# tigarcia/firedancer

Measured on AMD Instinct MI355X. Metric: ed25519 verifies/sec at 1/8 GPUs; % INT32 VALU roofline; p99 batch latency, higher is better.
Workload: dtype int32

## Files before the change

firedancer_amd/csrc/fd_ed25519_kernels.hip:

```cpp
#include <hip/hip_runtime.h>
#include "fd25519_dsm.h"
#include "fd25519_ge4.h"
#include "fd25519_sc.h"
#include "fd_sha512_dev.h"
#define FD_HALF_FN __device__ static inline
#define FD_HALF_RCP(y) __builtin_amdgcn_rcp(y)
#define FD_HALF_RCPF(y) __builtin_amdgcn_rcpf(y)
#include "fd25519_half.h"



#define FD_PF_FAIL  1u
#define FD_PF_SMALL 2u
#define FD_HF_DNEG  1u
#define FD_HF_FULL  2u


FD_DEV uint32_t nblk_bucket(uint32_t sz) {
  const uint32_t b = (sz + 208u) >> 7;
  return b < (FD_ED25519_SORT_BUCKETS - 1) ? b : (FD_ED25519_SORT_BUCKETS - 1);
}

#define FD_SORT_PER_THREAD 16
#define FD_SORT_PER_BLOCK (256 * FD_SORT_PER_THREAD)
// ... 108 lines not shown
  hash_finish(p, j, dig, S);
}

__global__ void __launch_bounds__(256, FD_ED25519_HASH_WAVES_PER_SIMD)
fd_ed25519_hash_kernel(fd_ed25519_verify_params_t p) {
  const uint64_t t = (uint64_t)blockIdx.x * blockDim.x + threadIdx.x;
  if (t >= p.n) return;
  hash_one(p, p.perm ? (uint64_t)p.perm[t] : t);
}

FD_DEV void decode_one(const fd_ed25519_verify_params_t& p, int which , uint64_t j) {
  const uint64_t i = p.base + j;
  uint32_t s[8];
  {
    const uint4* src = which ? reinterpret_cast<const uint4*>(p.sigs + 64 * i)
                             : reinterpret_cast<const uint4*>(p.pubs + 32 * i);
    const uint4 q0 = src[0], q1 = src[1];
    s[0] = q0.x; s[1] = q0.y; s[2] = q0.z; s[3] = q0.w; s[4] = q1.x; s[5] = q1.y; s[6] = q1.z; s[7] = q1.w;
  }
  decoded_pt d;
  ge_decode(d, s, !p.codes_portable);
  int32_t* dst = p.pts + (uint64_t)which * 20 * p.cap + j;
#pragma unroll
  for (int l = 0; l < 10; l++) {
    dst[(uint64_t)l * p.cap] = d.x.v[l];
    dst[(uint64_t)(10 + l) * p.cap] = d.y.v[l];
  }
  p.pflag[(uint64_t)which * p.cap + j] = (uint8_t)((d.fail ? FD_PF_FAIL : 0u) | (d.small ? FD_PF_SMALL : 0u));
}

__global__ void __launch_bounds__(256, FD_ED25519_DECODE_WAVES_PER_SIMD)
fd_ed25519_decode_kernel(fd_ed25519_verify_params_t p) {
  const uint64_t t = (uint64_t)blockIdx.x * blockDim.x + threadIdx.x;
  if (t >= 2 * p.n) return;
  const int which = t >= p.n;
  decode_one(p, which, which ? t - p.n : t);
}

FD_DEV void load_fe(fe& x, const int32_t* src, uint64_t cap) {
#pragma unroll
  for (int l = 0; l < 10; l++) x.v[l] = src[(uint64_t)l * cap];
}

FD_DEV void load_pt(fe& x, fe& y, const fd_ed25519_verify_params_t& p, int which, uint64_t j) {
  const int32_t* src = p.pts + (uint64_t)which * 20 * p.cap + j;
  load_fe(x, src, p.cap);
  load_fe(y, src + 10 * p.cap, p.cap);
}

#define FD_PENDING 1
FD_DEV int precheck(const fd_ed25519_verify_params_t& p, uint64_t j) {
  const uint32_t s_ok = p.sflag[j];
  const uint32_t af = p.pflag[j], rf = p.pflag[p.cap + j];
  if (!s_ok) return FD_ED25519_ERR_SIG;
  if (af & FD_PF_FAIL) return p.codes_portable ? FD_ED25519_ERR_PUBKEY : FD_ED25519_ERR_SIG;
  if (rf & FD_PF_FAIL) return FD_ED25519_ERR_SIG;
  if (af & FD_PF_SMALL) return FD_ED25519_ERR_PUBKEY;
  if (rf & FD_PF_SMALL) return FD_ED25519_ERR_SIG;
  return FD_PENDING;
}

template <bool NT>
FD_DEV void table_store(int4* tab, int e, ge_cached c) {
  if (NT) fe_neg(c.T2d, c.T2d);
  atab_store(tab, e, c);
}

__device__ const int4 fd_ident_cached[10] = {{1, 0, 0, 0}, {0, 0, 0, 0}, {0, 0, 1, 0}, {0, 0, 0, 0}, {0, 0, 0, 0},
                                             {2, 0, 0, 0}, {0, 0, 0, 0}, {0, 0, 0, 0}, {0, 0, 0, 0}, {0, 0, 0, 0}};

template <bool IDENT>
FD_DEV const int4* tab_entry(const int4* tab, int e) {
  const int a = e < 0 ? -e : e;
  if (IDENT) return a == 0 ? fd_ident_cached : tab + (a - 1) * 10;
  return tab + a * 10;
}

template <bool NT, bool IDENT = false>
FD_DEV void table_build(int4* tab, const fe& x, const fe& y, bool negate) {
  ge_p3 P0;
  fe xn;
  fe_neg(xn, x);
  fe_select(P0.X, x, xn, negate);
  P0.Y = y;
  fe_1(P0.Z);
  fe_mul(P0.T, P0.X, y);
  ge_cached c1, c;
  if (!IDENT) {
    c.YplusX = P0.Z; c.YminusX = P0.Z; fe_add(c.Z2, P0.Z, P0.Z); fe_0(c.T2d);
    atab_store(tab, 0, c);
  }
  ge_p3_to_cached(c1, P0);
  table_store<NT>(tab, IDENT ? 0 : 1, c1);
  ge_precomp pre;
  pre.yplusx = c1.YplusX; pre.yminusx = c1.YminusX; pre.xy2d = c1.T2d;
  ge_p3 cur = P0;
  ge_p1p1 sum;
#pragma clang loop unroll(disable)
  for (int e = 2; e <= 8; e++) {
    ge_madd(sum, cur, pre);
    ge_p1p1_to_p3_uxyt(cur, sum);
    ge_p3_to_cached<true>(c, cur);
    table_store<NT>(tab, IDENT ? e - 1 : e, c);
  }
}

FD_DEV void table_add(ge_p1p1& Rt, const ge_p3& P, const int4* tab, int e) {
  ge_cached c;
  atab_load(c, tab, e < 0 ? -e : e);
  ge_cached_cneg(c, e < 0);
  ge_add(Rt, P, c);
}

FD_DEV void btab_add(ge_p1p1& Rt, const ge_p3& P, ge_precomp& b, int f) {
  ge_precomp_cneg(b, f < 0);
  ge_madd(Rt, P, b);
}


FD_DEV bool half_pair_ok(const uint32_t (&k)[8], const uint32_t (&c)[FD_HALF_TW], const uint32_t (&dm)[FD_HALF_TW],
                         int dneg, int dbits) {
  uint32_t x[16];
#pragma unroll
  for (int w = 0; w < 16; w++) x[w] = 0u;
#pragma unroll
  for (int a = 0; a < FD_HALF_TW; a++) {
    uint64_t carry = 0;
#pragma unroll
    for (int b = 0; b < 8; b++) {
      const uint64_t t = (uint64_t)dm[a] * k[b] + x[a + b] + carry;
      x[a + b] = (uint32_t)t;
      carry = t >> 32;
    }
    x[a + 8] = (uint32_t)carry;
  }
  const uint32_t n8l[8] = FD_HALF_N8L;
  uint32_t add[8];
  {
    uint64_t br = 0;
#pragma unroll
    for (int w = 0; w < 8; w++) {
      const uint32_t cv = w < FD_HALF_TW ? c[w] : 0u;
      const uint64_t t = (uint64_t)n8l[w] - cv - br;
      br = (t >> 63) & 1u;
      add[w] = dneg ? cv : (uint32_t)t;
    }
  }
  {
    uint64_t carry = 0;
#pragma unroll
    for (int w = 0; w < 15; w++) {
      const uint64_t t = (uint64_t)x[w] + (w < 8 ? add[w] : 0u) + carry;
      x[w] = (uint32_t)t;
      carry = t >> 32;
    }
  }
  const uint32_t low = x[0] & 7u;
#pragma unroll
  for (int w = 0; w < 15; w++) x[w] = __builtin_amdgcn_alignbit(x[w + 1], x[w], 3);
  x[15] >>= 3;
  uint32_t r[8];
  sc_reduce512(r, x);
  uint32_t nz = low;
#pragma unroll
  for (int w = 0; w < 8; w++) nz |= r[w];
  return nz == 0u && (dm[0] & 1u) && fd_half_bitlen<FD_HALF_TW>(c) <= FD_HALF_BITS &&
         fd_half_bitlen<FD_HALF_TW>(dm) <= dbits;
}

#ifndef FD_ED25519_AB_LDS_BASE
#define FD_ED25519_AB_LDS_BASE 0
#endif
#ifndef FD_ED25519_HALF_FAULT
#define FD_ED25519_HALF_FAULT 0
#endif

FD_DEV int half_scalars_checked(const uint32_t (&k)[8], uint32_t (&c)[FD_HALF_TW], uint32_t (&dm)[FD_HALF_TW],
                                int* dneg, int dbits, uint64_t tag) {
  const int found = fd_half_scalars(k, c, dm, dneg, dbits);
#if FD_ED25519_HALF_FAULT
  {
    const uint32_t h = (uint32_t)(tag * 0x9E3779B97F4A7C15ull >> 32);
    const uint32_t sel = h >> 29, w = (h >> 8) & 3u, b = h & 31u;
#pragma unroll
    for (int i = 0; i < 4; i++) {
      if (sel == 1u && i == (int)w) c[i] ^= 1u << b;
      if (sel == 2u && i == (int)w) dm[i] ^= (i == 0 && b == 0) ? 2u : (1u << b);
    }
  }
#else
  (void)tag;
#endif
  return found && half_pair_ok(k, c, dm, *dneg, dbits);
}


FD_DEV void scalar_one(const fd_ed25519_verify_params_t& p, uint64_t j) {
  const uint64_t i = p.base + j;
  uint32_t k[8], S[8];
#pragma unroll
  for (int w = 0; w < 8; w++) k[w] = p.k[(uint64_t)w * p.cap + j];
  {
    const uint4* sg = reinterpret_cast<const uint4*>(p.sigs + 64 * i);
    const uint4 q2 = sg[2], q3 = sg[3];
    S[0] = q2.x; S[1] = q2.y; S[2] = q2.z; S[3] = q2.w; S[4] = q3.x; S[5] = q3.y; S[6] = q3.z; S[7] = q3.w;
  }
  uint32_t cw[FD_HALF_TW], dm[FD_HALF_TW];
  int dneg = 0;
  int ok = half_scalars_checked(k, cw, dm, &dneg, p.half_dbits, j);
  if (!p.sflag[j]) ok = 1;

  uint32_t sp[8];
  {
    uint32_t prod[16];
#pragma unroll
    for (int w = 0; w < 16; w++) prod[w] = 0u;
#pragma unroll
    for (int a = 0; a < FD_HALF_TW; a++) {
      uint64_t carry = 0;
#pragma unroll
      for (int b = 0; b < 8; b++) {
        const uint64_t t = (uint64_t)dm[a] * S[b] + prod[a + b] + carry;
        prod[a + b] = (uint32_t)t;
        carry = t >> 32;
      }
      prod[a + 8] = (uint32_t)carry;
    }
    sc_reduce512(sp, prod);
    if (dneg) {
      const uint32_t l[8] = {0x5cf5d3edu, 0x5812631au, 0xa2f79cd6u, 0x14def9deu, 0u, 0u, 0u, 0x10000000u};
      uint32_t nz = 0;
#pragma unroll
      for (int w = 0; w < 8; w++) nz |= sp[w];
      uint64_t br = 0;
#pragma unroll
      for (int w = 0; w < 8; w++) {
        const uint64_t t = (uint64_t)l[w] - sp[w] - br;
        br = (t >> 63) & 1u;
        sp[w] = nz ? (uint32_t)t : 0u;
      }
    }
  }
  uint32_t* hs = p.hs + j;
  const uint64_t c = p.cap;
  static_assert(FD_ED25519_BTABW_SHIFT == 144, "s_lo is words 0..3 and the low half of word 4");
#pragma unroll
  for (int w = 0; w < 5; w++) {
    hs[(uint64_t)w * c] = cw[w];
    hs[(uint64_t)(5 + w) * c] = dm[w];
    hs[(uint64_t)(10 + w) * c] = w < 4 ? sp[w] : (sp[4] & 0xffffu);
  }
#pragma unroll
  for (int w = 0; w < 4; w++)
    hs[(uint64_t)(15 + w) * c] = __builtin_amdgcn_alignbit(w + 5 < 8 ? sp[w + 5] : 0u, sp[w + 4], 16);
  p.hflag[j] = (uint8_t)((dneg ? FD_HF_DNEG : 0u) | (ok ? 0u : FD_HF_FULL));
  if (!ok && !p.small) {
    const uint32_t slot = atomicAdd(p.fix_cnt, 1u);
    p.fix_list[slot] = (uint32_t)j;
  }
}

__global__ void __launch_bounds__(256, FD_ED25519_SCALAR_WAVES_PER_SIMD)
fd_ed25519_scalar_kernel(fd_ed25519_verify_params_t p) {
  const uint64_t j = (uint64_t)blockIdx.x * blockDim.x + threadIdx.x;
  if (j >= p.n) return;
  scalar_one(p, j);
}

__global__ void __launch_bounds__(192) fd_ed25519_prep_kernel(fd_ed25519_verify_params_t p) {
  const uint32_t w = threadIdx.x >> 6;
  const uint64_t t = (uint64_t)blockIdx.x * 64u + (threadIdx.x & 63u);
  if (t >= p.n) return;
  if (w == 0) {
    const uint64_t j = p.perm ? (uint64_t)p.perm[t] : t;
    hash_one(p, j);
    scalar_one(p, j);
  } else {
    decode_one(p, (int)w - 1, t);
  }
}


FD_DEV void load_hs(uint32_t (&x)[5], const fd_ed25519_verify_params_t& p, int row, int words, uint64_t j) {
#pragma unroll
  for (int w = 0; w < 5; w++) x[w] = w < words ? p.hs[(uint64_t)(row + w) * p.cap + j] : 0u;
}

template <int BW>
struct fd_bw {
  static constexpr int STEP   = BW / 4;
  static constexpr int LO_N   = FD_ED25519_BTABW_SHIFT / BW;
  static constexpr int HI_N   = (253 - FD_ED25519_BTABW_SHIFT + BW - 1) / BW;
  static constexpr int LO_SHL = 160 - LO_N * BW;
  static constexpr int HI_SHL = 160 - HI_N * BW;
  static_assert(BW % 4 == 0, "base digits start at window boundaries");
  static_assert(LO_N * BW == FD_ED25519_BTABW_SHIFT, "s_lo digits cover bits 0..SHIFT-1");
  static_assert(HI_N * BW >= 253 - FD_ED25519_BTABW_SHIFT, "s_hi digits cover s' >> SHIFT");
  static_assert(STEP * (LO_N - 1) <= 32, "every base digit falls within the 33 windows");
  FD_DEV static bool lo_at(int it) { return it <= STEP * (LO_N - 1) && it % STEP == 0; }
  FD_DEV static bool hi_at(int it) { return it <= STEP * (HI_N - 1) && it % STEP == 0; }
};


template <int BW>
FD_DEV int dsm_half_one(const fd_ed25519_verify_params_t& p, uint64_t j, int4* tabA, int4* tabR) {
  int code = precheck(p, j);
  const uint32_t hf = p.hflag[j];

  {
    fe x, y;
    load_pt(x, y, p, 0, j);
    table_build<true, true>(tabA, x, y, true);
    load_pt(x, y, p, 1, j);
    table_build<true, true>(tabR, x, y, !(hf & FD_HF_DNEG));
  }
  uint32_t cd[5], dd[5], ld[5], hd[5];
  int W = 33;
  {
    uint32_t x[5], t[5];
    load_hs(x, p, 5, 5, j);
    const int wl = (fd_half_bitlen<5>(x) + 4) >> 2;
#pragma unroll
    for (int w = 34; w <= (FD_HALF_DBITS_MAX + 4) / 4; w++) W += __ballot(wl >= w) != 0ull;
    const int sh = 160 - 4 * W;
    shl160v(t, x, sh); recode160<4>(dd, t);
    load_hs(x, p, 0, 5, j);  shl160v(t, x, sh); recode160<4>(cd, t);
    load_hs(x, p, 10, 5, j); shl160<fd_bw<BW>::LO_SHL>(ld, x);
    load_hs(x, p, 15, 4, j); shl160<fd_bw<BW>::HI_SHL>(hd, x);
  }
  const int4* g_btab = reinterpret_cast<const int4*>(p.btab_lo);
  const int4* g_btab2 = reinterpret_cast<const int4*>(p.btab_hi);

  ge_p3 P;
  ge_p3_0(P);
  ge_p1p1 Rt;
  ge_p2 Q;
#pragma clang loop unroll(disable)
  for (int it = W - 1; it >= 0; it--) {
    int ea = pop160<4>(cd), er = pop160<4>(dd);
    if (it == W - 1) { ea &= 15; er &= 15; }
    ge_cached ca, cr;
    const bool blo = fd_bw<BW>::lo_at(it), bhi = fd_bw<BW>::hi_at(it);
    ge_precomp b1, b2;
    atab_load(ca, tab_entry<true>(tabA, ea), 0);
    if (it != W - 1) {
#pragma clang loop unroll(disable)
      for (int dbl = 0; dbl < 4; dbl++) {
        ge_p2_dbl(Rt, Q);
        if (dbl < 3) ge_p1p1_to_p2(Q, Rt);
      }
      ge_p1p1_to_p3_u(P, Rt);
    }
    atab_load(cr, tab_entry<true>(tabR, er), 0);
    ge_cached_cneg(ca, ea < 0);
    ge_add<true>(Rt, P, ca);
    ge_p1p1_to_p3_u(P, Rt);
    if (blo) btab16_load(b1, g_btab, (int)pop160u<BW>(ld));
    if (bhi) btab16_load(b2, g_btab2, (int)pop160u<BW>(hd));
    ge_cached_cneg(cr, er < 0);
    ge_add<true>(Rt, P, cr);
    if (blo) {
      ge_p1p1_to_p3_uxyt(P, Rt);
      ge_madd(Rt, P, b1);
    }
    if (bhi) {
      ge_p1p1_to_p3_uxyt(P, Rt);
      ge_madd(Rt, P, b2);
    }
    ge_p1p1_to_p2(Q, Rt);
  }
  fe t;
  fe_sub(t, Q.Y, Q.Z);
  const bool ident = fe_iszero(Q.X) && fe_iszero(t);
  if (code == FD_PENDING) code = ident ? FD_ED25519_SUCCESS : FD_ED25519_ERR_MSG;
  return code;
}

#if FD_ED25519_AB_LDS_BASE
FD_DEV int dsm_half_one_lds(const fd_ed25519_verify_params_t& p, uint64_t j, int4* tabA, int4* tabR,
                            const int4* s_lo8, const int4* s_hi8) {
  int code = precheck(p, j);
  const uint32_t hf = p.hflag[j];
  {
    fe x, y;
    load_pt(x, y, p, 0, j);
    table_build<true, true>(tabA, x, y, true);
    load_pt(x, y, p, 1, j);
    table_build<true, true>(tabR, x, y, !(hf & FD_HF_DNEG));
  }
  uint32_t cd[5], dd[5], ld[5], hd[5];
  int W = 33;
  {
    uint32_t x[5], t[5], sl[5], sh[5];
    load_hs(x, p, 5, 5, j);
    const int wl = (fd_half_bitlen<5>(x) + 4) >> 2;
#pragma unroll
    for (int w = 34; w <= (FD_HALF_DBITS_MAX + 4) / 4; w++) W += __ballot(wl >= w) != 0ull;
    const int shv = 160 - 4 * W;
    shl160v(t, x, shv); recode160<4>(dd, t);
    load_hs(x, p, 0, 5, j);  shl160v(t, x, shv); recode160<4>(cd, t);
    load_hs(sl, p, 10, 5, j);
    load_hs(sh, p, 15, 4, j);
    static_assert(FD_ED25519_BTABW_SHIFT - FD_ED25519_BTAB8_SHIFT == 8, "re-split of s' by one byte");
    uint32_t lo[5] = {sl[0], sl[1], sl[2], sl[3], sl[4] & 0xffu};
    uint32_t hi[5] = {(sl[4] >> 8) | (sh[0] << 8), (sh[0] >> 24) | (sh[1] << 8), (sh[1] >> 24) | (sh[2] << 8),
                      (sh[2] >> 24) | (sh[3] << 8), sh[3] >> 24};
    shl160<160 - 17 * 8>(ld, lo);
    shl160<160 - 15 * 8>(hd, hi);
  }
  ge_p3 P;
  ge_p3_0(P);
  ge_p1p1 Rt;
  ge_p2 Q;
#pragma clang loop unroll(disable)
  for (int it = W - 1; it >= 0; it--) {
    int ea = pop160<4>(cd), er = pop160<4>(dd);
    if (it == W - 1) { ea &= 15; er &= 15; }
    ge_cached ca, cr;
    const bool blo = it <= 32 && !(it & 1), bhi = it <= 28 && !(it & 1);
    ge_precomp b1, b2;
    atab_load(ca, tab_entry<true>(tabA, ea), 0);
    if (it != W - 1) {
#pragma clang loop unroll(disable)
      for (int dbl = 0; dbl < 4; dbl++) {
        ge_p2_dbl(Rt, Q);
        if (dbl < 3) ge_p1p1_to_p2(Q, Rt);
      }
      ge_p1p1_to_p3_u(P, Rt);
    }
    atab_load(cr, tab_entry<true>(tabR, er), 0);
    ge_cached_cneg(ca, ea < 0);
    ge_add<true>(Rt, P, ca);
    ge_p1p1_to_p3_u(P, Rt);
    if (blo) btab16_load(b1, s_lo8, (int)pop160u<8>(ld));
    if (bhi) btab16_load(b2, s_hi8, (int)pop160u<8>(hd));
    ge_cached_cneg(cr, er < 0);
    ge_add<true>(Rt, P, cr);
    if (blo) {
      ge_p1p1_to_p3_uxyt(P, Rt);
      ge_madd(Rt, P, b1);
    }
    if (bhi) {
      ge_p1p1_to_p3_uxyt(P, Rt);
      ge_madd(Rt, P, b2);
    }
    ge_p1p1_to_p2(Q, Rt);
  }
  fe t;
  fe_sub(t, Q.Y, Q.Z);
  const bool ident = fe_iszero(Q.X) && fe_iszero(t);
  if (code == FD_PENDING) code = ident ? FD_ED25519_SUCCESS : FD_ED25519_ERR_MSG;
  return code;
}
#endif

FD_DEV int dsm_full_core(const fd_ed25519_verify_params_t& p, uint64_t j, int4* tabA, int code, const fe& ax,
                         const fe& ay, const fe& rx, const fe& ry) {
  const uint64_t i = p.base + j;
  table_build<false>(tabA, ax, ay, true);
  uint32_t kd[8], sd[8];
  {
    uint32_t k[8], S[8];
#pragma unroll
    for (int w = 0; w < 8; w++) k[w] = p.k[(uint64_t)w * p.cap + j];
    const uint4* sg = reinterpret_cast<const uint4*>(p.sigs + 64 * i);
    const uint4 q2 = sg[2], q3 = sg[3];
    S[0] = q2.x; S[1] = q2.y; S[2] = q2.z; S[3] = q2.w; S[4] = q3.x; S[5] = q3.y; S[6] = q3.z; S[7] = q3.w;
    recode_radix16(kd, k);
    recode_radix65536(sd, S);
  }
  const int4* g_btab = reinterpret_cast<const int4*>(p.btab16);
  ge_p3 P;
  ge_p3_0(P);
  ge_p1p1 Rt;
  ge_p2 Q;
#pragma clang loop unroll(disable)
  for (int it = 63; it >= 0; it--) {
    const bool badd = (it & 3) == 0;
    int f = 0;
    ge_precomp b;
    if (badd) {
      f = pop_digit<16>(sd);
      btab16_load(b, g_btab, f < 0 ? -f : f);
    }
    if (it != 63) {
#pragma clang loop unroll(disable)
      for (int dbl = 0; dbl < 4; dbl++) {
        ge_p2_dbl(Rt, Q);
        if (dbl < 3) ge_p1p1_to_p2(Q, Rt);
      }
      ge_p1p1_to_p3_u(P, Rt);
    }
    table_add(Rt, P, tabA, pop_digit<4>(kd));
    if (badd) {
      ge_p1p1_to_p3_uxyt(P, Rt);
      btab_add(Rt, P, b, f);
    }
    ge_p1p1_to_p2(Q, Rt);
  }
  fe t1, t2;
  fe_mul(t1, rx, Q.Z);
  fe_sub(t1, t1, Q.X);
  fe_mul(t2, ry, Q.Z);
  fe_sub(t2, t2, Q.Y);
  const bool eq = fe_iszero(t1) && fe_iszero(t2);
  if (code != FD_PENDING) return code;
  return eq ? FD_ED25519_SUCCESS : FD_ED25519_ERR_MSG;
}

FD_DEV int dsm_full_one(const fd_ed25519_verify_params_t& p, uint64_t j, int4* tabA) {
  fe ax, ay, rx, ry;
  load_pt(ax, ay, p, 0, j);
  load_pt(rx, ry, p, 1, j);
  return dsm_full_core(p, j, tabA, precheck(p, j), ax, ay, rx, ry);
}

template <int BW>
__global__ void __launch_bounds__(FD_ED25519_VERIFY_BLOCK, FD_ED25519_DSM_WAVES_PER_SIMD)
fd_ed25519_dsm_kernel(fd_ed25519_verify_params_t p) {
  const uint32_t lane = threadIdx.x & 63u;
  const uint64_t wave = ((uint64_t)blockIdx.x * blockDim.x + threadIdx.x) >> 6;
  int4* tabA = reinterpret_cast<int4*>(static_cast<char*>(p.atab) + wave * FD_ED25519_ATAB_BYTES_PER_WAVE) +
               lane * (2 * FD_ED25519_ATAB_STRIDE * 10);
  int4* tabR = tabA + FD_ED25519_ATAB_STRIDE * 10;
#if FD_ED25519_AB_LDS_BASE
  __shared__ int4 s_b8[2 * 256 * (FD_ED25519_BTAB16_STRIDE / 4)];
  {
    const int4* g_lo = reinterpret_cast<const int4*>(p.btab8_lo);
    const int4* g_hi = reinterpret_cast<const int4*>(p.btab8_hi);
    constexpr int N = 256 * (FD_ED25519_BTAB16_STRIDE / 4);
    for (int i = threadIdx.x; i < N; i += blockDim.x) { s_b8[i] = g_lo[i]; s_b8[N + i] = g_hi[i]; }
    __syncthreads();
  }
#endif
  if (p.small) {
    const uint64_t stride = (uint64_t)gridDim.x * blockDim.x;
    for (uint64_t t = (uint64_t)blockIdx.x * blockDim.x + threadIdx.x; t < p.n; t += stride)
      if (p.hflag[t] & FD_HF_FULL) p.out[p.base + t] = (int8_t)dsm_full_one(p, t, tabA);
    return;
  }
  const uint64_t nfix = *p.fix_cnt;
  const uint64_t head = (nfix + 63u) & ~(uint64_t)63u;
  const uint64_t total = head + p.n;
  for (;;) {
    uint32_t b = 0u;
    if (lane == 0u) b = atomicAdd(p.work_ctr, 64u);
    b = (uint32_t)__builtin_amdgcn_readfirstlane((int)__shfl((int)b, 0));
    if ((uint64_t)b >= total) break;
    const uint64_t t = (uint64_t)b + lane;
    if (t < nfix) {
      const uint64_t j = p.fix_list[t];
      p.out[p.base + j] = (int8_t)dsm_full_one(p, j, tabA);
    } else if (t >= head && t < total) {
      const uint64_t j = t - head;
#if FD_ED25519_AB_LDS_BASE
      if (!(p.hflag[j] & FD_HF_FULL))
        p.out[p.base + j] = (int8_t)dsm_half_one_lds(p, j, tabA, tabR, s_b8, s_b8 + 256 * (FD_ED25519_BTAB16_STRIDE / 4));
#else
      if (!(p.hflag[j] & FD_HF_FULL)) p.out[p.base + j] = (int8_t)dsm_half_one<BW>(p, j, tabA, tabR);
#endif
    }
  }
}


FD_DEV void tab4_store(int4* tab, int e, const fe& c) {
  int4* d = tab + 3 * e;
  d[0] = make_int4(c.v[0], c.v[1], c.v[2], c.v[3]);
  d[1] = make_int4(c.v[4], c.v[5], c.v[6], c.v[7]);
  d[2] = make_int4(c.v[8], c.v[9], 0, 0);
}

FD_DEV void tab4_load(fe& c, const int4* tab, int e) {
  const int4* s = tab + 3 * e;
  const int4 a = s[0], b = s[1], d = s[2];
  c.v[0] = a.x; c.v[1] = a.y; c.v[2] = a.z; c.v[3] = a.w;
  c.v[4] = b.x; c.v[5] = b.y; c.v[6] = b.z; c.v[7] = b.w;
  c.v[8] = d.x; c.v[9] = d.y;
}

FD_DEV void btab4_load(fe& c, const int32_t* g_btab, int e, const qmask_t& m) {
  const int off = m.l0 ? 10 : (m.l1 ? 0 : 20);
  const int2* s = reinterpret_cast<const int2*>(g_btab + (size_t)e * FD_ED25519_BTAB16_STRIDE + off);
#pragma unroll
  for (int q = 0; q < 5; q++) {
    const int2 x = s[q];
    c.v[2 * q] = x.x;
    c.v[2 * q + 1] = x.y;
  }
#pragma unroll
  for (int i = 0; i < 10; i++) c.v[i] = m.l3 ? (i == 0 ? 2 : 0) : c.v[i];
}

FD_DEV void table4_build(int4* tab, const fe& x, const fe& y, bool negate, const qmask_t& m) {
  fe xs, xy, p0, c1, c, r, cur;
#pragma unroll
  for (int i = 0; i < 10; i++) xs.v[i] = negate ? -x.v[i] : x.v[i];
  fe_mul(xy, xs, y);
#pragma unroll
  for (int i = 0; i < 10; i++) {
    p0.v[i] = m.l0 ? xs.v[i] : (m.l1 ? y.v[i] : (m.l2 ? (i == 0 ? 1 : 0) : xy.v[i]));
    c.v[i] = i == 0 ? (m.l2 ? 0 : (m.l3 ? 2 : 1)) : 0;
  }
  tab4_store(tab, 0, c);
  ge4_to_qc(c1, p0, m);
  tab4_store(tab, 1, c1);
  cur = p0;
#pragma clang loop unroll(disable)
  for (int e = 2; e <= 8; e++) {
    ge4_add(r, cur, c1, m);
    ge4_to_p3(cur, r);
    ge4_to_qc(c, cur, m);
    tab4_store(tab, e, c);
  }
}

template <int BW>
__global__ void __launch_bounds__(256) fd_ed25519_dsm4_kernel(fd_ed25519_verify_params_t p) {
  const uint64_t gid = (uint64_t)blockIdx.x * blockDim.x + threadIdx.x;
  const uint64_t j = gid >> 2;
  if (j >= p.n) return;
  const uint32_t hf = p.hflag[j];
  if (hf & FD_HF_FULL) return;
  const qmask_t m = quad_masks();
  int4* tabA = reinterpret_cast<int4*>(static_cast<char*>(p.atab) + gid * FD_ED25519_QUAD_LANE_BYTES);
  int4* tabR = tabA + 27;
  int code = precheck(p, j);
  {
    fe x, y;
    load_pt(x, y, p, 0, j);
    table4_build(tabA, x, y, true, m);
    load_pt(x, y, p, 1, j);
    table4_build(tabR, x, y, !(hf & FD_HF_DNEG), m);
  }
  uint32_t cd[5], dd[5], ld[5], hd[5];
  int W = 33;
  {
    uint32_t x[5], t[5];
    load_hs(x, p, 5, 5, j);
    const int wl = (fd_half_bitlen<5>(x) + 4) >> 2;
#pragma unroll
    for (int w = 34; w <= (FD_HALF_DBITS_MAX + 4) / 4; w++) W += __ballot(wl >= w) != 0ull;
    const int sh = 160 - 4 * W;
    shl160v(t, x, sh); recode160<4>(dd, t);
    load_hs(x, p, 0, 5, j);  shl160v(t, x, sh); recode160<4>(cd, t);
    load_hs(x, p, 10, 5, j); shl160<fd_bw<BW>::LO_SHL>(ld, x);
    load_hs(x, p, 15, 4, j); shl160<fd_bw<BW>::HI_SHL>(hd, x);
  }
  fe P, Rt;
#pragma unroll
  for (int i = 0; i < 10; i++) P.v[i] = (i == 0 && (m.l1 | m.l2)) ? 1 : 0;
#pragma clang loop unroll(disable)
  for (int it = W - 1; it >= 0; it--) {
    int ea = pop160<4>(cd), er = pop160<4>(dd);
    if (it == W - 1) { ea &= 15; er &= 15; }
    const bool blo = fd_bw<BW>::lo_at(it), bhi = fd_bw<BW>::hi_at(it);
    fe ca, cr, b1, b2;
    tab4_load(ca, tabA, ea < 0 ? -ea : ea);
    if (it != W - 1) {
#pragma clang loop unroll(disable)
      for (int dbl = 0; dbl < 4; dbl++) {
        ge4_dbl(Rt, P, m);
        ge4_to_p3(P, Rt);
      }
    }
    tab4_load(cr, tabR, er < 0 ? -er : er);
    ge4_cneg(P, m.l03, ea < 0);
    ge4_add(Rt, P, ca, m);
    ge4_cneg(Rt, m.l0, ea < 0);
    ge4_to_p3(P, Rt);
    if (blo) btab4_load(b1, p.btab_lo, (int)pop160u<BW>(ld), m);
    if (bhi) btab4_load(b2, p.btab_hi, (int)pop160u<BW>(hd), m);
    ge4_cneg(P, m.l03, er < 0);
    ge4_add(Rt, P, cr, m);
    ge4_cneg(Rt, m.l0, er < 0);
    ge4_to_p3(P, Rt);
    if (blo) {
      ge4_add(Rt, P, b1, m);
      ge4_to_p3(P, Rt);
    }
    if (bhi) {
      ge4_add(Rt, P, b2, m);
      ge4_to_p3(P, Rt);
    }
  }
  fe y1, z1, t;
  fe_qp<FD_QP(1, 1, 1, 1)>(y1, P);
  fe_qp<FD_QP(2, 2, 2, 2)>(z1, P);
  fe_sub(t, y1, z1);
  const bool ident = fe_iszero(P) && fe_iszero(t);
  if (code == FD_PENDING) code = ident ? FD_ED25519_SUCCESS : FD_ED25519_ERR_MSG;
  if (m.l0) p.out[p.base + j] = (int8_t)code;
}

template <int BW>
__global__ void __launch_bounds__(256) fd_ed25519_dsm8_kernel(fd_ed25519_verify_params_t p) {
  const uint64_t gid = (uint64_t)blockIdx.x * blockDim.x + threadIdx.x;
  const uint64_t j = gid >> 3;
  if (j >= p.n) return;
  const uint32_t hf = p.hflag[j];
  if (hf & FD_HF_FULL) return;
  const int half = (int)((threadIdx.x >> 2) & 1u);
  const qmask_t m = quad_masks();
  int4* tab = reinterpret_cast<int4*>(static_cast<char*>(p.atab) + gid * (FD_ED25519_QUAD_LANE_BYTES / 2));
  int code = precheck(p, j);
  {
    fe x, y;
    load_pt(x, y, p, half, j);
    table4_build(tab, x, y, half ? !(hf & FD_HF_DNEG) : true, m);
  }
  uint32_t sd[5], bd[5];
  int W = 33;
  {
    uint32_t x[5], t[5];
    load_hs(x, p, 5, 5, j);
    const int wl = (fd_half_bitlen<5>(x) + 4) >> 2;
#pragma unroll
    for (int w = 34; w <= (FD_HALF_DBITS_MAX + 4) / 4; w++) W += __ballot(wl >= w) != 0ull;
    if (!half) load_hs(x, p, 0, 5, j);
    shl160v(t, x, 160 - 4 * W); recode160<4>(sd, t);
    if (half) {
      load_hs(x, p, 15, 4, j);
      shl160<fd_bw<BW>::HI_SHL>(bd, x);
    } else {
      load_hs(x, p, 10, 5, j);
      shl160<fd_bw<BW>::LO_SHL>(bd, x);
    }
  }
  const int32_t* btab = half ? p.btab_hi : p.btab_lo;
  fe P, Rt;
#pragma unroll
  for (int i = 0; i < 10; i++) P.v[i] = (i == 0 && (m.l1 | m.l2)) ? 1 : 0;
#pragma clang loop unroll(disable)
  for (int it = W - 1; it >= 0; it--) {
    int e = pop160<4>(sd);
    if (it == W - 1) e &= 15;
    const bool badd = half ? fd_bw<BW>::hi_at(it) : fd_bw<BW>::lo_at(it);
    fe ce, b;
    tab4_load(ce, tab, e < 0 ? -e : e);
    if (it != W - 1) {
#pragma clang loop unroll(disable)
      for (int dbl = 0; dbl < 4; dbl++) {
        ge4_dbl(Rt, P, m);
        ge4_to_p3(P, Rt);
      }
    }
    if (badd) btab4_load(b, btab, (int)pop160u<BW>(bd), m);
    ge4_cneg(P, m.l03, e < 0);
    ge4_add(Rt, P, ce, m);
    ge4_cneg(Rt, m.l0, e < 0);
    ge4_to_p3(P, Rt);
    if (badd) {
      ge4_add(Rt, P, b, m);
      ge4_to_p3(P, Rt);
    }
  }
  fe q, qs;
  ge4_to_qc(q, P, m);
#pragma unroll
  for (int i = 0; i < 10; i++) qs.v[i] = __shfl_down(q.v[i], 4);
  ge4_add(Rt, P, qs, m);
  ge4_to_p3(P, Rt);
  fe y1, z1, t;
  fe_qp<FD_QP(1, 1, 1, 1)>(y1, P);
  fe_qp<FD_QP(2, 2, 2, 2)>(z1, P);
  fe_sub(t, y1, z1);
  const bool ident = fe_iszero(P) && fe_iszero(t);
  if (code == FD_PENDING) code = ident ? FD_ED25519_SUCCESS : FD_ED25519_ERR_MSG;
  if (m.l0 && !half) p.out[p.base + j] = (int8_t)code;
}

#include "fd25519_r16.h"

FD_DEV fe btab16_fetch(const int32_t* g_btab, int e, const r16ctx& k) {
  const int off = (int)((k.r0 & 10u) | (k.r2 & 20u));
  const int2* src = reinterpret_cast<const int2*>(g_btab + (size_t)e * FD_ED25519_BTAB16_STRIDE + off);
  fe c;
#pragma unroll
  for (int q = 0; q < 5; q++) {
    const int2 x = src[q];
    c.v[2 * q] = x.x;
    c.v[2 * q + 1] = x.y;
  }
  return c;
}
FD_DEV uint32_t btab16_r16(const fe& c, const r16ctx& k) {
  return (r16_from_fe(c, k) & ~k.r3) | (r16_small(2u, k) & k.r3);
}

FD_DEV uint32_t wait_go(const uint32_t* go) {
  for (uint32_t spin = 0u; spin < FD_ED25519_GO_SPIN_MAX; spin++) {
    const uint32_t g = __hip_atomic_load(go, __ATOMIC_RELAXED, __HIP_MEMORY_SCOPE_SYSTEM);
    if (g != 0u) {
      __atomic_thread_fence(__ATOMIC_ACQUIRE);
      return g;
    }
    __builtin_amdgcn_s_sleep(8);
  }
  return 0u;
}

template <int BW>
__global__ void __launch_bounds__(128) fd_ed25519_dsm16_kernel(fd_ed25519_verify_params_t p) {
  const uint64_t j = blockIdx.x;
  if (j >= p.n) return;
  if (p.go) {
    __shared__ uint32_t go;
    if (threadIdx.x == 0u) go = wait_go(p.go);
    __syncthreads();
    if (go != FD_ED25519_GO_RUN) return;
  }
  const uint32_t hf = p.hflag[j];
  const int half = (int)(threadIdx.x >> 6);
  uint32_t hd[5], hx[5], hb[5];
  load_hs(hd, p, 5, 5, j);
  load_hs(hx, p, half ? 5 : 0, 5, j);
  load_hs(hb, p, half ? 15 : 10, half ? 4 : 5, j);
  if (hf & FD_HF_FULL) return;
  r16ctx k;
  r16_init(k);
  const uint32_t d2 = r16_from_fe(fe{FE_D2}, k);
  uint32_t tab[9];
  {
    fe x, y;
    load_pt(x, y, p, half, j);
    table16_build(tab, r16_from_fe(x, k), r16_from_fe(y, k), half ? !(hf & FD_HF_DNEG) : true, d2, k);
  }
  uint32_t sd[5], bd[5];
  int W = 33;
  {
    uint32_t t[5];
    W = (fd_half_bitlen<5>(hd) + 4) >> 2;
    W = W < 33 ? 33 : W;
    shl160v(t, hx, 160 - 4 * W); recode160<4>(sd, t);
    if (half) shl160<fd_bw<BW>::HI_SHL>(bd, hb);
    else      shl160<fd_bw<BW>::LO_SHL>(bd, hb);
  }
  W = __builtin_amdgcn_readfirstlane(W);
  const int32_t* btab = half ? p.btab_hi : p.btab_lo;
  const uint32_t one = r16_small(1u, k);
  uint32_t P = one & k.r12;
#pragma clang loop unroll(disable)
  for (int it = W - 1; it >= 0; it--) {
    int e = pop160<4>(sd);
    if (it == W - 1) e &= 15;
    e = __builtin_amdgcn_readfirstlane(e);
    const bool badd = half ? fd_bw<BW>::hi_at(it) : fd_bw<BW>::lo_at(it);
    const uint32_t bdig = (uint32_t)__builtin_amdgcn_readfirstlane((int)(badd ? pop160u<BW>(bd) : 0u));
    const uint32_t ce = table16_at(tab, e < 0 ? -e : e);
    fe braw;
    if (badd) braw = btab16_fetch(btab, (int)bdig, k);
    if (it != W - 1) {
      P = ge16_dbl2<false, false>(P, k);
      P = ge16_dbl2<true, false>(P, k);
      P = ge16_dbl2<true, false>(P, k);
      P = ge16_dbl2<true, true>(P, k);
    }
    uint32_t b = 0u;
    if (badd) b = btab16_r16(braw, k);
    if (e != 0) {
      P = ge16_cneg4(P, k.r03, e < 0, k);
      P = ge16_add2<true>(P, ce, e < 0, k);
// ... 608 lines not shown
```

Baseline: 104.5 million.

## Use joint A/R Straus table with 2-bit windows in half-size DSM

Replaces the two separate per-point 4-bit window tables for A and R with one joint table of combined a*A+r*R entries for signed 2-bit digits, built with shared-difference additions. The main loop then takes twice as many windows with 2 doublings each but only one cached addition per window instead of two, and sign symmetry halves the table size. The aim is to cut point additions in the variable-base part, at the cost of a more complex table build and per-step digit-pair sign normalization.

Result: faster. 106.1 million (median of 6 runs) (+1.5%).

```diff
diff --git a/firedancer_amd/csrc/fd_ed25519_kernels.hip b/firedancer_amd/csrc/fd_ed25519_kernels.hip
--- a/firedancer_amd/csrc/fd_ed25519_kernels.hip
+++ b/firedancer_amd/csrc/fd_ed25519_kernels.hip
@@ -434,29 +434,97 @@
 };
 
 
+FD_DEV void jtab_store(int4* tab, int slot, const ge_p3& P, bool neg) {
+  ge_cached c;
+  ge_p3_to_cached<true>(c, P);
+  fe_neg(c.T2d, c.T2d);
+  ge_cached_cneg(c, neg);
+  atab_store(tab, slot, c);
+}
+
+FD_DEV void jtab_affine(ge_p3& P, const fd_ed25519_verify_params_t& p, int which, uint64_t j, bool negate) {
+  fe x, xn;
+  load_pt(x, P.Y, p, which, j);
+  fe_neg(xn, x);
+  fe_select(P.X, x, xn, negate);
+  fe_1(P.Z);
+  fe_mul(P.T, P.X, P.Y);
+}
+
+FD_DEV void jtab_step(int4* tab, int src, const ge_p3& q, int sp, int sm, bool mneg) {
+  ge_cached e;
+  atab_load(e, tab, src);
+  fe qs, qd, m;
+  fe_add(qs, q.Y, q.X);
+  fe_sub(qd, q.Y, q.X);
+  fe_mul(m, e.T2d, q.T);
+#pragma clang loop unroll(disable)
+  for (int h = sm < 0 ? 1 : 0; h < 2; h++) {
+    const bool plus = h != 0;
+    fe u, v, a, b, ms, mn;
+    fe_select(u, qd, qs, plus);
+    fe_select(v, qs, qd, plus);
+    fe_mul_u(a, e.YplusX, u);
+    fe_mul_u(b, e.YminusX, v);
+    fe_neg(mn, m);
+    fe_select(ms, mn, m, plus);
+    ge_p1p1 sum;
+    fe_sub(sum.X, a, b);
+    fe_add(sum.Y, a, b);
+    fe_sub(sum.Z, e.Z2, ms);
+    fe_add(sum.T, e.Z2, ms);
+    ge_p3 K;
+    ge_p1p1_to_p3_uxyt(K, sum);
+    jtab_store(tab, plus ? sp : sm, K, !plus && mneg);
+  }
+}
+
+#define FD_JSLOT(a, r) (5 * (a) + (r) - 1)
+FD_DEV void joint_table_build(int4* tab, const fd_ed25519_verify_params_t& p, uint64_t j, bool rneg) {
+  ge_p3 P;
+#pragma clang loop unroll(disable)
+  for (int w = 0; w < 2; w++) {
+    jtab_affine(P, p, w, j, w ? rneg : true);
+    ge_cached c1;
+    ge_p3_to_cached(c1, P);
+    table_store<true>(tab, w ? FD_JSLOT(0, 1) : FD_JSLOT(1, 0), c1);
+    ge_p1p1 sum;
+    ge_p3_dbl(sum, P);
+    ge_p3 D;
+    ge_p1p1_to_p3_uxyt(D, sum);
+    jtab_store(tab, w ? FD_JSLOT(0, 2) : FD_JSLOT(2, 0), D, false);
+  }
+#pragma clang loop unroll(disable)
+  for (int st = 0; st < 4; st++) {
+    const int src = st == 0 ? FD_JSLOT(0, 2) : st == 1 ? FD_JSLOT(1, 0) : st == 2 ? FD_JSLOT(2, 0) : FD_JSLOT(2, 1);
+    const int sp = st == 0 ? FD_JSLOT(1, 2) : st == 1 ? FD_JSLOT(1, 1) : st == 2 ? FD_JSLOT(2, 1) : FD_JSLOT(2, 2);
+    const int sm = st == 0 ? FD_JSLOT(1, -2) : st == 1 ? FD_JSLOT(1, -1) : st == 2 ? FD_JSLOT(2, -1) : -1;
+    jtab_affine(P, p, st ? 1 : 0, j, st ? rneg : true);
+    jtab_step(tab, src, P, sp, sm, st == 0);
+  }
+}
+
+FD_DEV const int4* jtab_entry(const int4* tab, int a, int r) {
+  const int slot = FD_JSLOT(a, r);
+  return slot < 0 ? fd_ident_cached : tab + slot * 10;
+}
+
 template <int BW>
-FD_DEV int dsm_half_one(const fd_ed25519_verify_params_t& p, uint64_t j, int4* tabA, int4* tabR) {
+FD_DEV int dsm_half_one(const fd_ed25519_verify_params_t& p, uint64_t j, int4* tab) {
   int code = precheck(p, j);
   const uint32_t hf = p.hflag[j];
-
-  {
-    fe x, y;
-    load_pt(x, y, p, 0, j);
-    table_build<true, true>(tabA, x, y, true);
-    load_pt(x, y, p, 1, j);
-    table_build<true, true>(tabR, x, y, !(hf & FD_HF_DNEG));
-  }
+  joint_table_build(tab, p, j, !(hf & FD_HF_DNEG));
   uint32_t cd[5], dd[5], ld[5], hd[5];
-  int W = 33;
+  int W = 66;
   {
     uint32_t x[5], t[5];
     load_hs(x, p, 5, 5, j);
-    const int wl = (fd_half_bitlen<5>(x) + 4) >> 2;
-#pragma unroll
-    for (int w = 34; w <= (FD_HALF_DBITS_MAX + 4) / 4; w++) W += __ballot(wl >= w) != 0ull;
-    const int sh = 160 - 4 * W;
-    shl160v(t, x, sh); recode160<4>(dd, t);
-    load_hs(x, p, 0, 5, j);  shl160v(t, x, sh); recode160<4>(cd, t);
+    const int wl = (fd_half_bitlen<5>(x) + 2) >> 1;
+#pragma unroll
+    for (int w = 67; w <= (FD_HALF_DBITS_MAX + 2) / 2; w++) W += __ballot(wl >= w) != 0ull;
+    const int sh = 160 - 2 * W;
+    shl160v(t, x, sh); recode160<2>(dd, t);
+    load_hs(x, p, 0, 5, j);  shl160v(t, x, sh); recode160<2>(cd, t);
     load_hs(x, p, 10, 5, j); shl160<fd_bw<BW>::LO_SHL>(ld, x);
     load_hs(x, p, 15, 4, j); shl160<fd_bw<BW>::HI_SHL>(hd, x);
   }
@@ -464,33 +532,37 @@
   const int4* g_btab2 = reinterpret_cast<const int4*>(p.btab_hi);
 
   ge_p3 P;
-  ge_p3_0(P);
   ge_p1p1 Rt;
   ge_p2 Q;
+  {
+    const int ea = pop160<2>(cd) & 3, er = pop160<2>(dd) & 3;
+    ge_cached cj;
+    atab_load(cj, jtab_entry(tab, ea, er), 0);
+    fe t;
+    fe_sub(t, cj.YplusX, cj.YminusX);
+    fe_carry(Q.X, t);
+    fe_add(t, cj.YplusX, cj.YminusX);
+    fe_carry(Q.Y, t);
+    Q.Z = cj.Z2;
+  }
 #pragma clang loop unroll(disable)
-  for (int it = W - 1; it >= 0; it--) {
-    int ea = pop160<4>(cd), er = pop160<4>(dd);
-    if (it == W - 1) { ea &= 15; er &= 15; }
-    ge_cached ca, cr;
-    const bool blo = fd_bw<BW>::lo_at(it), bhi = fd_bw<BW>::hi_at(it);
+  for (int it = W - 2; it >= 0; it--) {
+    const int ea = pop160<2>(cd), er = pop160<2>(dd);
+    const bool sg = ea < 0 || (ea == 0 && er < 0);
+    ge_cached cj;
+    const bool blo = !(it & 1) && fd_bw<BW>::lo_at(it >> 1), bhi = !(it & 1) && fd_bw<BW>::hi_at(it >> 1);
     ge_precomp b1, b2;
-    atab_load(ca, tab_entry<true>(tabA, ea), 0);
-    if (it != W - 1) {
-#pragma clang loop unroll(disable)
-      for (int dbl = 0; dbl < 4; dbl++) {
-        ge_p2_dbl(Rt, Q);
-        if (dbl < 3) ge_p1p1_to_p2(Q, Rt);
-      }
-      ge_p1p1_to_p3_u(P, Rt);
-    }
-    atab_load(cr, tab_entry<true>(tabR, er), 0);
-    ge_cached_cneg(ca, ea < 0);
-    ge_add<true>(Rt, P, ca);
-    ge_p1p1_to_p3_u(P, Rt);
+    atab_load(cj, jtab_entry(tab, sg ? -ea : ea, sg ? -er : er), 0);
     if (blo) btab16_load(b1, g_btab, (int)pop160u<BW>(ld));
     if (bhi) btab16_load(b2, g_btab2, (int)pop160u<BW>(hd));
-    ge_cached_cneg(cr, er < 0);
-    ge_add<true>(Rt, P, cr);
+#pragma clang loop unroll(disable)
+    for (int dbl = 0; dbl < 2; dbl++) {
+      ge_p2_dbl(Rt, Q);
+      if (dbl < 1) ge_p1p1_to_p2(Q, Rt);
+    }
+    ge_p1p1_to_p3_u(P, Rt);
+    ge_cached_cneg(cj, sg);
+    ge_add<true>(Rt, P, cj);
     if (blo) {
       ge_p1p1_to_p3_uxyt(P, Rt);
       ge_madd(Rt, P, b1);
@@ -654,8 +726,8 @@
   const uint64_t wave = ((uint64_t)blockIdx.x * blockDim.x + threadIdx.x) >> 6;
   int4* tabA = reinterpret_cast<int4*>(static_cast<char*>(p.atab) + wave * FD_ED25519_ATAB_BYTES_PER_WAVE) +
                lane * (2 * FD_ED25519_ATAB_STRIDE * 10);
+#if FD_ED25519_AB_LDS_BASE
   int4* tabR = tabA + FD_ED25519_ATAB_STRIDE * 10;
-#if FD_ED25519_AB_LDS_BASE
   __shared__ int4 s_b8[2 * 256 * (FD_ED25519_BTAB16_STRIDE / 4)];
   {
     const int4* g_lo = reinterpret_cast<const int4*>(p.btab8_lo);
@@ -689,7 +761,7 @@
       if (!(p.hflag[j] & FD_HF_FULL))
         p.out[p.base + j] = (int8_t)dsm_half_one_lds(p, j, tabA, tabR, s_b8, s_b8 + 256 * (FD_ED25519_BTAB16_STRIDE / 4));
 #else
-      if (!(p.hflag[j] & FD_HF_FULL)) p.out[p.base + j] = (int8_t)dsm_half_one<BW>(p, j, tabA, tabR);
+      if (!(p.hflag[j] & FD_HF_FULL)) p.out[p.base + j] = (int8_t)dsm_half_one<BW>(p, j, tabA);
 #endif
     }
   }
```
